# apple/ml-unigen

Measured on AMD Instinct MI355X. Metric: train-step samples/s (1.5B, 256^2 img), higher is better.
Workload: dtype bf16

## Files before the change

include/unigen_hip.h:

```cpp
#ifndef UNIGEN_HIP_H
#define UNIGEN_HIP_H

#include <stdint.h>
#include <hip/hip_runtime_api.h>

#ifdef __cplusplus
extern "C" {
#endif

#define UG_ABI_VERSION 7

const char* ug_last_error(void);
int ug_abi_version(void);

typedef struct ug_handle ug_handle;
int ug_create(ug_handle** out);
int ug_destroy(ug_handle* h);

#define UG_EPI_BF16 0
#define UG_EPI_F32 1
#define UG_EPI_RESID 2
int ug_gemm_bf16(const ug_handle* h, const void* A, int64_t lda, int a_kmajor, const void* B, int64_t ldb, int b_kmajor,
                 void* C, int64_t ldc, int64_t M, int64_t N, int64_t K, int epilogue, const void* bias,
                 const float* resid, int64_t ldr, int beta, const float* alpha_dev, int policy, hipStream_t stream);
#define UG_GEMM_NARROW_EPILOGUE 0x100
#define UG_GEMM_ONE_BARRIER 0x200
#define UG_GEMM_TWO_BARRIERS 0x400
#define UG_GEMM_POLICY_AUTO_BITS 0xff

int ug_cast_f32_bf16(const float* in, void* out, int64_t n, hipStream_t stream);

int ug_gemm_bf16_swiglu_bwd(const ug_handle* h, const void* dy, int64_t ld_dy, const void* w_down, int64_t ldw, const void* gu,
                            int64_t ld_gu, void* dgu, int64_t ld_dgu, int64_t M, int64_t I, int64_t K, hipStream_t stream);
int ug_gemm_set_fused_tile_height(int rows);
int ug_gemm_bf16_qkv_rope(const ug_handle* h, const void* x, int64_t ldx, const void* w, int64_t ldw, const void* bias, void* qkv,
                          int64_t ldq, int64_t M, int64_t N, int64_t K, const float* cos_tab, const float* sin_tab, int64_t L,
                          int64_t rope_cols, int head_dim, hipStream_t stream);
int ug_gemm_bf16_swiglu(const ug_handle* h, const void* x, int64_t ldx, const void* w_gate_up, int64_t ldw, void* gu,
                        int64_t ld_gu, void* act, int64_t ld_act, int64_t M, int64_t I, int64_t K, hipStream_t stream);

int ug_gemm_bf16_wgrad_group(int n, const void* const* dy, const int64_t* ld_dy, const void* const* x, const int64_t* ld_x,
                             float* const* dw, const int64_t* ld_dw, const int64_t* rows, const int64_t* cols,
                             const int* beta, const int64_t* K, hipStream_t stream);

int ug_rmsnorm_fwd(const float* x, const float* w, void* y, float* rstd, int64_t rows, int64_t cols,
                   float eps, int out_f32, hipStream_t stream);
int ug_rmsnorm_bwd(const void* dy, const float* x, const float* rstd, const float* w, float* dres,
                   float* dw, void* dres_bf16, int64_t rows, int64_t cols, hipStream_t stream);
int ug_rope(void* qkv, const float* cos_tab, const float* sin_tab, int64_t tokens, int64_t L, int64_t ldq,
            int nheads, int head_dim, int backward, hipStream_t stream);
int ug_swiglu_fwd(const void* gate_up, void* act, int64_t tokens, int64_t I, hipStream_t stream);
int ug_swiglu_bwd(const void* gate_up, const void* dact, void* dgate_up, int64_t tokens, int64_t I,
                  hipStream_t stream);
int ug_gelu(const void* x, const void* dy_or_null, void* out, int64_t n, hipStream_t stream);
int ug_embed_fwd(const int64_t* ids, const float* W, float* out, int64_t tokens, int64_t H, int64_t V,
                 int* err_flag, hipStream_t stream);
int ug_embed_bwd(const int64_t* ids, const float* dout, float* dW, int64_t tokens, int64_t H, int64_t V,
                 hipStream_t stream);
int ug_embed_bwd_sorted(const int64_t* ids_sorted, const int64_t* order, const float* rows, float* dW, int64_t n,
                        int64_t H, int64_t V, float scale, hipStream_t stream);
int ug_gather_rows_bf16(const void* in, int64_t ld_in, const int64_t* idx, void* out, int64_t ld_out,
                        int64_t n, int64_t C, int scatter, hipStream_t stream);
int ug_colsum_bf16(const void* in, int64_t ld, float* out, int64_t R, int64_t C, hipStream_t stream);

#define UG_MASK_F32 0
#define UG_MASK_BF16 1
#define UG_MASK_I64 2
// ... 215 lines not shown
```

ml-unigen_amd/csrc/gemm_bf16.hip:

```cpp
#include "common.h"
#include <type_traits>
#include <atomic>
#include "unigen_hip.h"
#include "vmem_asm.h"
#include "gemm_plan.h"

namespace {

using namespace ug_plan;
constexpr int TILE_BYTES = BM * BK * 2;
constexpr int GROUP_M = 8;
constexpr int P8_GROUP_M = 4;

typedef const __attribute__((address_space(1))) void* gptr_t;
typedef __attribute__((address_space(3))) void* lptr_t;
typedef __attribute__((ext_vector_type(4))) short s16x4_t;

__device__ __attribute__((aligned(16))) uint32_t g_zero_page[64];

struct GemmArgs {
  const bf16_t* A; const bf16_t* B; void* C;
  const bf16_t* bias;
  const float* resid;
  const float* alpha_dev;
  int M, N, K;
  int64_t lda, ldb, ldc, ldr;
  int beta;
  const bf16_t* sw_gu; int64_t ld_gu;
  const float* rope_cos; const float* rope_sin; int rope_L, rope_cols;
  int tiles_m, tiles_n;
  int full_tiles, tail_split;
  float* tail_ws;
  int tail_private;
  int one_barrier;
  int wide_epilogue;
  int swiglu_I;
  bf16_t* act; int64_t ld_act;
};
// ... 770 lines not shown
      if constexpr (decltype(steady)::value) {
        stage_in(t + 3);
        landed(2);
      } else {
        if (t + 3 < nk) stage_in(t + 3);
        landed(min(nk - 1, t + 3) - (t + 1));
      }
      asm volatile("s_waitcnt lgkmcnt(0)" ::: "memory");
      P_BARRIER();
      __builtin_amdgcn_s_setprio(1);
      UG_MFMA_BLOCK(FG)
      __builtin_amdgcn_s_setprio(0);
      P_BARRIER();
    };
    int t = 0;
    for (; t + 4 < nk; ++t) iteration(t, std::true_type{});
    for (; t < nk; ++t) iteration(t, std::false_type{});
    if (G0) P_BARRIER();
    if constexpr (EPI == EPI_SWIGLU_BWD)
      store_tile_swiglu_bwd<FG>(p, reinterpret_cast<f32x4_t (&)[FG][4]>(acc[0]), lds + wave * EP_STRIP, m0 + (G0 ? 0 : 16 * F0), n0 + wn * 64, lane);
    else if constexpr (EPI == EPI_SWIGLU)
      store_tile_swiglu_perm<FG>(p, reinterpret_cast<f32x4_t (&)[FG][4]>(acc[0]), lds + wave * EP_STRIP, m0 + (G0 ? 0 : 16 * F0), tn * 128 + wn * 32, lane);
    else if constexpr (EPI == EPI_ROPE)
      store_tile_lds<EPI, FG>(p, reinterpret_cast<f32x4_t (&)[FG][4]>(acc[0]), lds + wave * EP_STRIP, m0 + (G0 ? 0 : 16 * F0),
                              n0 + (wn >> 1) * 128 + (wn & 1) * 32, lane, (wn & 1) * 32, n0 < p.rope_cols);
    else
      store_tile_lds<EPI, FG>(p, reinterpret_cast<f32x4_t (&)[FG][4]>(acc[0]), lds + wave * EP_STRIP, m0 + (G0 ? 0 : 16 * F0), n0 + wn * 64, lane);
  };
  const bool more = REM != 0 && wave < REM;
  if (grp == 0) { if (more) run(std::true_type{}, std::integral_constant<int, LO + (REM ? 1 : 0)>{}); else run(std::true_type{}, std::integral_constant<int, LO>{}); }
  else { if (more) run(std::false_type{}, std::integral_constant<int, LO + (REM ? 1 : 0)>{}); else run(std::false_type{}, std::integral_constant<int, LO>{}); }
}


template <int EPI>
__global__ __launch_bounds__(256) void tail_finish_kernel(GemmArgs p, int ntail) {
  const int nwg = p.tiles_m * p.tiles_n;
  const int per_tile = PBM * PBN / 4;
  const int64_t total = (int64_t)ntail * per_tile;
  float alpha = 1.f;
  if constexpr (EPI == EPI_F32) { if (p.alpha_dev) alpha = *p.alpha_dev; }
  for (int64_t idx = blockIdx.x * (int64_t)blockDim.x + threadIdx.x; idx < total; idx += (int64_t)gridDim.x * blockDim.x) {
    const int tl = (int)(idx / per_tile), q = (int)(idx % per_tile);
    const int pid = xcd_remap(p.full_tiles + tl, nwg);
    const int per_group = P8_GROUP_M * p.tiles_n;
    const int gid = pid / per_group, first_m = gid * P8_GROUP_M;
    const int gsz = min(p.tiles_m - first_m, P8_GROUP_M);
    const int tm = first_m + (pid % per_group) % gsz;
    const int tn = (pid % per_group) / gsz;
    const int ml = q / (PBN / 4), nl = (q % (PBN / 4)) * 4;
    float4 v4;
    if (p.tail_private) {
      const int nk_all = (p.K + PBK - 1) / PBK, per_split = (nk_all + p.tail_split - 1) / p.tail_split;
      v4 = make_float4(0.f, 0.f, 0.f, 0.f);
      for (int sp = 0; sp < p.tail_split && sp * per_split < nk_all; ++sp) {
        const float4 t = *reinterpret_cast<const float4*>(p.tail_ws + ((int64_t)tl * p.tail_split + sp) * (PBM * PBN) + ml * PBN + nl);
        v4.x += t.x; v4.y += t.y; v4.z += t.z; v4.w += t.w;
      }
    } else {
      float4* src = reinterpret_cast<float4*>(p.tail_ws + (int64_t)tl * (PBM * PBN) + ml * PBN + nl);
      v4 = *src;
      *src = make_float4(0.f, 0.f, 0.f, 0.f);
    }
    const int m = tm * PBM + ml, n = tn * PBN + nl;
    if (m >= p.M || n >= p.N) continue;
    float v[4] = {v4.x, v4.y, v4.z, v4.w};
    for (int r = 0; r < 4 && n + r < p.N; ++r) {
      if constexpr (EPI == EPI_BF16) {
        float o = v[r];
        if (p.bias) o += bf2f(p.bias[n + r]);
        reinterpret_cast<bf16_t*>(p.C)[(int64_t)m * p.ldc + n + r] = f2bf(o);
      } else if constexpr (EPI == EPI_F32) {
        float* c = reinterpret_cast<float*>(p.C) + (int64_t)m * p.ldc + n + r;
        *c = (p.beta ? *c : 0.f) + v[r] * alpha;
      } else {
        reinterpret_cast<float*>(p.C)[(int64_t)m * p.ldc + n + r] = p.resid[(int64_t)m * p.ldr + n + r] + bf2f(f2bf(v[r]));
      }
    }
  }
}

static_assert(WS_PRIVATE_SLOTS == UG_HANDLE_WS_SLOTS && POLICY_NARROW_EPILOGUE == UG_GEMM_NARROW_EPILOGUE && POLICY_ONE_BARRIER == UG_GEMM_ONE_BARRIER &&
              POLICY_TWO_BARRIERS == UG_GEMM_TWO_BARRIERS && POLICY_AUTO_BITS == UG_GEMM_POLICY_AUTO_BITS, "gemm_plan.h restates these");

bool env_switch_on(const char* name) { const char* v = getenv(name); return !(v && atoi(v) == 0); }

template <int EPI, bool BKM, int H>
bool launch_p10_height(int height, dim3 grid, const GemmArgs& a, hipStream_t st) {
  if (height != H) return false;
  hipLaunchKernelGGL((gemm_kernel_p10<EPI, BKM, p10_f0(H), p10_f1(H)>), grid, dim3(512), 0, st, a);
  return true;
}
template <int EPI, bool BKM, int... H>
bool launch_p10(HeightList<H...>, int height, dim3 grid, const GemmArgs& a, hipStream_t st) {
  return (launch_p10_height<EPI, BKM, H>(height, grid, a, st) || ...);
}

template <int EPI, bool AK, bool BKM>
int run_plan(const GemmPlan& pl, GemmArgs a, hipStream_t st) {
  a.tiles_m = pl.tiles_m; a.tiles_n = pl.tiles_n;
  a.full_tiles = pl.full_tiles; a.tail_split = pl.tail_split; a.tail_private = pl.tail_private;
  if (!pl.uses_workspace) a.tail_ws = nullptr;
  const dim3 grid(pl.grid_x, pl.grid_y);
  if (pl.kind == KIND_P10) {
    if constexpr (!AK && EPI != EPI_F32) {
      if (launch_p10<EPI, BKM>(typename P10Heights<EPI>::type{}, pl.height, grid, a, st)) {
        UG_CHECK_LAUNCH("ug_gemm_bf16(p10)");
        return UG_OK;
      }
    }
    ug_set_error("ug_gemm_bf16: no %d-row tile kernel for this layout and epilogue", pl.height);
    return UG_ERR_ARG;
  }
  if (pl.kind == KIND_128) {
    if (pl.dbuf) hipLaunchKernelGGL((gemm_kernel<EPI, AK, BKM, true>), grid, dim3(256), 0, st, a);
    else hipLaunchKernelGGL((gemm_kernel<EPI, AK, BKM, false>), grid, dim3(256), 0, st, a);
    UG_CHECK_LAUNCH("ug_gemm_bf16");
    return UG_OK;
  }
  const bool sliced = pl.kind == KIND_256_SLICED;
  if (a.one_barrier) hipLaunchKernelGGL((gemm_kernel_p8<EPI, AK, BKM, true>), grid, dim3(512), 0, st, a);
  else hipLaunchKernelGGL((gemm_kernel_p8<EPI, AK, BKM>), grid, dim3(512), 0, st, a);
  UG_CHECK_LAUNCH(sliced ? "ug_gemm_bf16(p8 k-sliced)" : "ug_gemm_bf16(p8)");
  if (pl.finish_tiles) {
    hipLaunchKernelGGL((tail_finish_kernel<EPI>), dim3(pl.finish_tiles * 16), dim3(256), 0, st, a, pl.finish_tiles);
    UG_CHECK_LAUNCH(sliced ? "ug_gemm_bf16(partial sum)" : "ug_gemm_bf16(tail finish)");
  }
  return UG_OK;
}

std::atomic<int> g_fused_height{0};

template <int EPI, bool BKM>
int launch_fused(GemmArgs a, int64_t col_tiles, const char* who, hipStream_t st) {
  const int forced = g_fused_height.load();
  const int hb = plan_fused(EPI, a.M, col_tiles, forced);
  if (hb < 0) {
    ug_set_error("%s: tile height %d forced by ug_gemm_set_fused_tile_height is not instantiated for this epilogue", who, forced);
    return UG_ERR_ARG;
  }
  a.tiles_m = (a.M + hb - 1) / hb; a.tiles_n = (int)col_tiles;
  a.tail_split = 1; a.tail_private = 1; a.wide_epilogue = 1;
  launch_p10<EPI, BKM>(typename P10Heights<EPI>::type{}, hb, dim3(a.tiles_m * a.tiles_n), a, st);
  UG_CHECK_LAUNCH(who);
  return UG_OK;
}

}

extern "C" int ug_gemm_bf16(const ug_handle* h, const void* A, int64_t lda, int a_kmajor, const void* B, int64_t ldb, int b_kmajor,
                            void* C, int64_t ldc, int64_t M, int64_t N, int64_t K, int epilogue, const void* bias,
                            const float* resid, int64_t ldr, int beta, const float* alpha_dev, int policy, hipStream_t stream) {
  UG_REQUIRE(M > 0 && N > 0 && K > 0, "ug_gemm_bf16: empty problem M=%ld N=%ld K=%ld", (long)M, (long)N, (long)K);
  UG_REQUIRE(lda % 8 == 0 && ldb % 8 == 0, "ug_gemm_bf16: lda/ldb must be multiples of 8 elements (16-byte rows)");
  UG_REQUIRE(ug_aligned16(A) && ug_aligned16(B) && ug_aligned16(C), "ug_gemm_bf16: A/B/C must be 16-byte aligned");
  UG_REQUIRE(ldc % 4 == 0, "ug_gemm_bf16: ldc must be a multiple of 4 elements");
  UG_REQUIRE(M < (1 << 30) && N < (1 << 30) && K < (1 << 30), "ug_gemm_bf16: dims too large");
  UG_REQUIRE(a_kmajor || b_kmajor || K % 8 == 0,
             "ug_gemm_bf16: K=%ld must be a multiple of 8 when both operands are row-major", (long)K);
  UG_REQUIRE(a_kmajor || lda >= ((K + 7) & ~7LL), "ug_gemm_bf16: row-major A needs lda >= round_up(K,8)");
  UG_REQUIRE(b_kmajor || ldb >= ((K + 7) & ~7LL), "ug_gemm_bf16: row-major B needs ldb >= round_up(K,8)");
  UG_REQUIRE(!a_kmajor || lda >= M, "ug_gemm_bf16: k-major A needs lda >= M");
  UG_REQUIRE(!b_kmajor || ldb >= N, "ug_gemm_bf16: k-major B needs ldb >= N");
  if (epilogue == EPI_RESID) UG_REQUIRE(resid != nullptr && ldr % 4 == 0, "ug_gemm_bf16: EPI_RESID needs a 16B-aligned residual");
  const GemmPolicy pol = decode_policy(policy, a_kmajor != 0, b_kmajor != 0);
  GemmArgs a{};
  a.A = (const bf16_t*)A; a.B = (const bf16_t*)B; a.C = C;
  a.bias = (const bf16_t*)bias; a.resid = resid; a.alpha_dev = alpha_dev;
  a.M = (int)M; a.N = (int)N; a.K = (int)K;
  a.lda = lda; a.ldb = ldb; a.ldc = ldc; a.ldr = ldr; a.beta = beta;
  a.wide_epilogue = pol.wide_epilogue; a.one_barrier = pol.one_barrier;
  a.tail_ws = h ? h->tail_ws : nullptr;
  static const bool heights_on = env_switch_on("UNIGEN_GEMM_HEIGHTS");
  GemmProblem pr;
  pr.M = a.M; pr.N = a.N; pr.K = a.K; pr.epilogue = epilogue; pr.a_kmajor = a_kmajor != 0; pr.b_kmajor = b_kmajor != 0; pr.beta = beta;
  pr.ldc = ldc; pr.ldr = ldr; pr.bias_aligned8 = !bias || (reinterpret_cast<uintptr_t>(bias) & 7) == 0;
  pr.has_workspace = a.tail_ws != nullptr; pr.policy = pol.policy; pr.heights_on = heights_on;
  const GemmPlan pl = plan_gemm(pr);
  const int mode = (a_kmajor ? 2 : 0) | (b_kmajor ? 1 : 0);
  switch (mode * 4 + epilogue) {
    case 0 * 4 + EPI_BF16: return run_plan<EPI_BF16, false, false>(pl, a, stream);
    case 0 * 4 + EPI_F32: return run_plan<EPI_F32, false, false>(pl, a, stream);
    case 0 * 4 + EPI_RESID: return run_plan<EPI_RESID, false, false>(pl, a, stream);
    case 1 * 4 + EPI_BF16: return run_plan<EPI_BF16, false, true>(pl, a, stream);
    case 1 * 4 + EPI_F32: return run_plan<EPI_F32, false, true>(pl, a, stream);
    case 3 * 4 + EPI_F32: return run_plan<EPI_F32, true, true>(pl, a, stream);
    case 3 * 4 + EPI_BF16: return run_plan<EPI_BF16, true, true>(pl, a, stream);
    default:
      ug_set_error("ug_gemm_bf16: layout/epilogue combination (a_kmajor=%d b_kmajor=%d epilogue=%d) is not instantiated",
                   a_kmajor, b_kmajor, epilogue);
      return UG_ERR_ARG;
  }
}

extern "C" int ug_gemm_bf16_wgrad_group(int n, const void* const* dy, const int64_t* ld_dy, const void* const* x, const int64_t* ld_x,
                                        float* const* dw, const int64_t* ld_dw, const int64_t* rows, const int64_t* cols,
                                        const int* beta, const int64_t* K, hipStream_t stream) {
  UG_REQUIRE(n >= 1 && n <= GROUP_MAX && K, "ug_gemm_bf16_wgrad_group: 1..%d problems and their contraction lengths required", GROUP_MAX);
  GroupArgs g;
  g.n = n;
  int start = 0;
  for (int i = 0; i < n; ++i) {
    UG_REQUIRE(rows[i] > 0 && cols[i] > 0 && rows[i] < (1 << 30) && cols[i] < (1 << 30) && K[i] > 0 && K[i] < (1 << 30),
               "ug_gemm_bf16_wgrad_group: empty problem %d", i);
    UG_REQUIRE(ld_dy[i] % 8 == 0 && ld_x[i] % 8 == 0 && ld_dy[i] >= rows[i] && ld_x[i] >= cols[i] && ld_dw[i] % 4 == 0 && ld_dw[i] >= cols[i],
               "ug_gemm_bf16_wgrad_group: problem %d: token-major operands need leading dimensions that are multiples of 8 and cover "
               "their rows; ld_dw a multiple of 4", i);
    UG_REQUIRE(ug_aligned16(dy[i]) && ug_aligned16(x[i]) && ug_aligned16(dw[i]), "ug_gemm_bf16_wgrad_group: problem %d: 16-byte alignment", i);
    GroupProblem& pr = g.pr[i];
    pr.A = (const bf16_t*)dy[i]; pr.B = (const bf16_t*)x[i]; pr.C = dw[i];
    pr.lda = ld_dy[i]; pr.ldb = ld_x[i]; pr.ldc = ld_dw[i];
    pr.M = (int)rows[i]; pr.N = (int)cols[i]; pr.K = (int)K[i]; pr.beta = beta[i];
    pr.tiles_m = (pr.M + PBM - 1) / PBM; pr.tiles_n = (pr.N + PBN - 1) / PBN;
    pr.start = start;
    start += (pr.tiles_m * pr.tiles_n + 7) & ~7;
  }
  for (int i = n; i < GROUP_MAX; ++i) { g.pr[i] = g.pr[0]; g.pr[i].start = 1 << 30; }
  hipLaunchKernelGGL(gemm_kernel_p8_wgrad_group, dim3(start), dim3(512), 0, stream, g);
  UG_CHECK_LAUNCH("ug_gemm_bf16_wgrad_group");
  return UG_OK;
}

extern "C" int ug_gemm_set_fused_tile_height(int rows) {
  UG_REQUIRE(rows == 0 || (rows >= 128 && rows <= 320 && rows % 16 == 0), "ug_gemm_set_fused_tile_height: 0 (automatic) or 128 ... 320 in steps of 16 (%d)", rows);
  g_fused_height.store(rows);
  return UG_OK;
}

extern "C" int ug_swiglu_fwd(const void* gate_up, void* act, int64_t tokens, int64_t I, hipStream_t st);

extern "C" int ug_gemm_bf16_swiglu(const ug_handle* h, const void* x, int64_t ldx, const void* w_gate_up, int64_t ldw, void* gu,
                                   int64_t ld_gu, void* act, int64_t ld_act, int64_t M, int64_t I, int64_t K, hipStream_t stream) {
  UG_REQUIRE(M > 0 && I > 0 && K > 0 && K % 8 == 0 && I % 8 == 0, "ug_gemm_bf16_swiglu: bad problem M=%ld I=%ld K=%ld", (long)M, (long)I, (long)K);
  UG_REQUIRE(ldx % 8 == 0 && ldw % 8 == 0 && ld_gu % 8 == 0 && ld_act % 8 == 0 && ldx >= K && ldw >= K && ld_gu >= 2 * I && ld_act >= I,
             "ug_gemm_bf16_swiglu: row strides must be multiples of 8 elements and cover the rows");
  UG_REQUIRE(ug_aligned16(x) && ug_aligned16(w_gate_up) && ug_aligned16(gu) && ug_aligned16(act), "ug_gemm_bf16_swiglu: alignment");
  UG_REQUIRE(M < (1 << 30) && I < (1 << 29) && K < (1 << 30), "ug_gemm_bf16_swiglu: dims too large");
  const int64_t tiles = ((M + PBM - 1) / PBM) * (2 * I / PBN);
  if (I % 128 != 0 || tiles < 64 || K % PBK != 0 || 2 * I / PBN > (1 << 20)) {
    if (int rc = ug_gemm_bf16(h, x, ldx, 0, w_gate_up, ldw, 0, gu, ld_gu, M, 2 * I, K, EPI_BF16, nullptr, nullptr, 0, 0, nullptr, -1, stream))
      return rc;
    UG_REQUIRE(ld_gu == 2 * I && ld_act == I, "ug_gemm_bf16_swiglu: the two-launch form needs packed gu / act rows");
    return ug_swiglu_fwd(gu, act, M, I, stream);
  }
  GemmArgs a{};
  a.A = (const bf16_t*)x; a.B = (const bf16_t*)w_gate_up; a.C = gu;
  a.M = (int)M; a.N = (int)(2 * I); a.K = (int)K;
  a.lda = ldx; a.ldb = ldw; a.ldc = ld_gu;
  a.swiglu_I = (int)I; a.act = (bf16_t*)act; a.ld_act = ld_act;
  return launch_fused<EPI_SWIGLU, false>(a, 2 * I / PBN, "ug_gemm_bf16_swiglu", stream);
}

extern "C" int ug_rope(void* qkv, const float* cos_tab, const float* sin_tab, int64_t tokens, int64_t L, int64_t ldq,
                       int nheads, int head_dim, int backward, hipStream_t st);

extern "C" int ug_gemm_bf16_qkv_rope(const ug_handle* h, const void* x, int64_t ldx, const void* w, int64_t ldw, const void* bias, void* qkv,
                                     int64_t ldq, int64_t M, int64_t N, int64_t K, const float* cos_tab, const float* sin_tab, int64_t L,
                                     int64_t rope_cols, int head_dim, hipStream_t stream) {
  UG_REQUIRE(M > 0 && N > 0 && K > 0 && L > 0 && M % L == 0 && head_dim > 0 && rope_cols >= 0 && rope_cols <= N && rope_cols % head_dim == 0,
             "ug_gemm_bf16_qkv_rope: bad problem M=%ld N=%ld K=%ld L=%ld rope_cols=%ld head_dim=%d", (long)M, (long)N, (long)K, (long)L,
             (long)rope_cols, head_dim);
// ... 35 lines not shown
```

ml-unigen_amd/csrc/gemm_plan.h:

```cpp
#pragma once
#include <cstdint>

namespace ug_plan {

enum Epi { EPI_BF16 = 0, EPI_F32 = 1, EPI_RESID = 2, EPI_ROPE = 3, EPI_SWIGLU = 4, EPI_SWIGLU_BWD = 5 };

constexpr int BM = 128, BN = 128, BK = 64;
constexpr int PBM = 256, PBN = 256, PBK = 32;
constexpr int QBM = 320;
constexpr int WS_PRIVATE_SLOTS = 768;

constexpr int imin(int a, int b) { return a < b ? a : b; }
constexpr int imax(int a, int b) { return a > b ? a : b; }

constexpr int POLICY_NARROW_EPILOGUE = 0x100, POLICY_ONE_BARRIER = 0x200, POLICY_TWO_BARRIERS = 0x400, POLICY_AUTO_BITS = 0xff;

struct GemmPolicy {
  int policy;
  bool one_barrier;
  bool wide_epilogue;
};

inline GemmPolicy decode_policy(int policy, bool a_kmajor, bool b_kmajor) {
  GemmPolicy d;
  d.wide_epilogue = !(policy >= 0 && (policy & POLICY_NARROW_EPILOGUE));
  d.one_barrier = a_kmajor && b_kmajor;
  if (policy >= 0 && (policy & POLICY_ONE_BARRIER)) d.one_barrier = true;
  if (policy >= 0 && (policy & POLICY_TWO_BARRIERS)) d.one_barrier = false;
  if (policy >= 0) policy &= ~(POLICY_NARROW_EPILOGUE | POLICY_ONE_BARRIER | POLICY_TWO_BARRIERS);
  if (policy == POLICY_AUTO_BITS) policy = -1;
  d.policy = policy;
  return d;
}

constexpr int p10_f0(int h) { return (h / 16 + 1) / 2; }
constexpr int p10_f1(int h) { return (h / 16) / 2; }

template <int... H>
struct HeightList {
  static constexpr int count = sizeof...(H);
  static constexpr int values[sizeof...(H)] = {H...};
};
template <int EPI> struct P10Heights { using type = HeightList<128, 144, 160, 176, 192, 208, 224, 240, 256, 272, 288, 304, 320>; };
template <> struct P10Heights<EPI_ROPE> { using type = HeightList<128, 160, 192, 208, 224, 256, 288, 320>; };
template <> struct P10Heights<EPI_SWIGLU> { using type = HeightList<128, 160, 192, 208, 224, 256, 288, 320>; };
template <> struct P10Heights<EPI_SWIGLU_BWD> { using type = HeightList<128, 160, 192, 208, 224, 256, 272, 288, 320>; };

struct GemmProblem {
  int M, N, K;
  int epilogue;
  bool a_kmajor, b_kmajor;
  int beta;
  int64_t ldc, ldr;
  bool bias_aligned8;
  bool has_workspace;
  int policy;
  bool heights_on;
};

enum GemmKind { KIND_128 = 0, KIND_256 = 1, KIND_256_SLICED = 2, KIND_P10 = 3 };

struct GemmPlan {
// ... 140 lines not shown
```

ml-unigen_amd/unigen_hip/lib.py:

```python
import ctypes
import os
import subprocess

_HERE = os.path.dirname(os.path.abspath(__file__))
CSRC_DIR = os.path.normpath(os.path.join(_HERE, "..", "csrc"))
LIB_PATH = os.environ.get("UNIGEN_HIP_LIB") or os.path.join(CSRC_DIR, "libunigen_hip.so")

ABI_VERSION = 7
P = ctypes.c_void_p
I64 = ctypes.c_int64
I32 = ctypes.c_int
F32 = ctypes.c_float

SIGNATURES = {
    "ug_abi_version": [],
    "ug_create": [P],
    "ug_destroy": [P],
    "ug_gemm_bf16": [P, P, I64, I32, P, I64, I32, P, I64, I64, I64, I64, I32, P, P, I64, I32, P, I32, P],
    "ug_gemm_bf16_qkv_rope": [P, P, I64, P, I64, P, P, I64, I64, I64, I64, P, P, I64, I64, I32, P],
    "ug_gemm_bf16_swiglu_bwd": [P, P, I64, P, I64, P, I64, P, I64, I64, I64, I64, P],
    "ug_gemm_bf16_swiglu": [P, P, I64, P, I64, P, I64, P, I64, I64, I64, I64, P],
    "ug_cast_f32_bf16": [P, P, I64, P],
    "ug_rmsnorm_fwd": [P, P, P, P, I64, I64, F32, I32, P],
    "ug_rmsnorm_bwd": [P, P, P, P, P, P, P, I64, I64, P],
    "ug_rope": [P, P, P, I64, I64, I64, I32, I32, I32, P],
    "ug_swiglu_fwd": [P, P, I64, I64, P],
    "ug_swiglu_bwd": [P, P, P, I64, I64, P],
    "ug_gelu": [P, P, P, I64, P],
    "ug_embed_fwd": [P, P, P, I64, I64, I64, P, P],
    "ug_embed_bwd": [P, P, P, I64, I64, I64, P],
    "ug_embed_bwd_sorted": [P, P, P, P, I64, I64, I64, F32, P],
    "ug_gather_rows_bf16": [P, I64, P, P, I64, I64, I64, I32, P],
    "ug_colsum_bf16": [P, I64, P, I64, I64, P],
    "ug_attn_mask_compress": [P, I32, I64, I64, P, P, I64, I64, P, P],
    "ug_attn_mask_causal": [P, P, P, I64, I64, P],
    "ug_attn_fwd": [P, P, P, I64, P, I64, P, P, P, I64, I64, I64, I32, I32, I32, F32, P],
    "ug_attn_bwd": [P, P, P, I64, P, P, I64, P, P, P, P, P, I64, P, P, I64, I64, I64, I32, I32, I32, F32, P, P, P, P, P],
    "ug_kv_store": [P, I64, I64, I64, P, P, I64, I64, I32, I32, I64, P, I32, P],
    "ug_rope_at": [P, P, P, I64, I64, I32, I32, P, I64, P],
    "ug_attn_decode": [P, I64, P, P, P, P, I64, I64, I32, I32, I32, I64, P, F32, P],
    "ug_gemv_bf16": [P, I64, I64, P, I64, P, I64, I64, I64, I64, P],
    "ug_decode_gemv": [P, I64, I64, P, I64, P, I64, I64, I64, P, I64, P, I64, P, P],
    "ug_decode_gemv_resid_norm": [P, P, I64, P, P, P, I64, P, I64, P, I64, I64, I64, P, I64, P, I64, P, P],
    "ug_decode_gemv_swiglu": [P, I64, P, F32, I64, I64, P, I64, P, I64, I64, I64, P, I64, P, I64, P, P],
    "ug_gemm_set_fused_tile_height": [I32],
    "ug_attn_decode_fused": [P, I64, P, F32, I64, P, P, P, P, P, P, P, P, I64, I64, I32, I32, I32, I64, I64, F32, P],
    "ug_decode_finish_resid_norm": [P, I64, P, P, P, I64, I64, F32, P, P, P],
    "ug_decode_sw_supported": [I64, I64, I64, I32],
    "ug_decode_sw_kblock": [P, I64, I64, P, I64, P, I64, I64, I64, P, I64, P, I64, P, P],
    "ug_decode_sw_resid": [P, I64, I64, P, I64, I64, I64, P, P],
    "ug_decode_sw_gate_up": [P, P, I64, P, P, F32, I64, I64, P, I64, I64, P, I64, P],
    "ug_decode_sw_head": [P, P, I64, P, P, F32, I64, I64, P, I64, I64, P, I64, P, P, P],
    "ug_t2i_assemble": [P, P, P, I64, P, I64, P, P, I64, I64, I64, I64, I64, I64, I64, P, P, P, P],
    "ug_attn_mask_from_ids": [P, I64, I64, I64, I64, I64, I32, P, P, P, P, P],
    "ug_maskgit_train_mask": [P, P, P, I64, I64, I64, I64, P, P, P],
    "ug_ar_sample": [P, I64, I64, I64, F32, F32, I32, P, P, I64, I64, P, I64, I64, I64, P, P, P, P],
    "ug_ar_sample_filtered": [P, I64, I64, I64, F32, F32, I32, P, P, I64, I64, P, I64, I64, I64, P, P, P, I64, F32, F32, P, P],
    "ug_text_pick": [P, I64, I64, I64, I32, P, I64, I64, P, I64, I64, I64, P, I64, P, P, P, P, P],
    "ug_text_sample_workspace_ints": [I64],
    "ug_text_sample": [P, I64, I64, I64, I32, F32, I64, F32, P, P, P, P, I64, I64, P, I64, I64, I64, P, I64, P, P, P, P, P],
    "ug_ar_sample_logp": [P, I64, I64, I64, F32, F32, I32, P, P, I64, I64, P, I64, I64, I64, P, P, P, P, P],
    "ug_ar_sample_filtered_logp": [P, I64, I64, I64, F32, F32, I32, P, P, I64, I64, P, I64, I64, I64, P, P, P, I64, F32, F32, P, P, P],
    "ug_text_pick_logp": [P, I64, I64, I64, I32, P, I64, I64, P, I64, I64, I64, P, I64, P, P, P, P, P, P],
    "ug_text_sample_logp": [P, I64, I64, I64, I32, F32, I64, F32, P, P, P, P, I64, I64, P, I64, I64, I64, P, I64, P, P, P, P, P, P],
    "ug_text_seen_mark": [P, I64, P, I64, I64, I64, P, I64, P],
    "ug_text_penalize": [P, I64, I64, I64, F32, P, I64, P, P],
    "ug_maskgit_step": [P, I64, I64, I64, I64, I32, F32, P, P, P, I64, I64, I64, F32, P, P, P, P, P, P],
    "ug_skinny_finish": [P, P, P, P, I64, I64, I32, P],
    "ug_gemv_bf16_ord": [P, I64, I64, P, I64, P, I64, I64, I64, I64, P],
    "ug_skinny_finish_ord": [P, I64, I64, P, P, P, P, I64, I64, P],
    "ug_decode_gemv_resid_norm_ord": [P, P, I64, I64, P, P, P, I64, P, I64, P, I64, I64, I64, P],
    "ug_attn_decode_fused_ord": [P, I64, I64, P, F32, I64, P, P, P, P, P, P, P, P, I64, I64, I32, I32, I32, I64, I64, F32, P],
    "ug_decode_sw_kblock_ord": [P, I64, I64, P, I64, P, I64, I64, I64, P],
    "ug_decode_finish_resid_norm_ord": [P, I64, I64, P, P, P, I64, I64, F32, P, P, P],
    "ug_ce_fwd": [P, I64, I64, I64, P, I64, P, P, P, P, P],
    "ug_ce_bwd": [P, I64, I64, I64, P, I64, P, P, P, P, P],
    "ug_adamw_flat": [P, P, P, P, P, I64, F32, F32, F32, F32, F32, I64, F32, I32, P],
    "ug_gemm_bf16_wgrad_group": [I32, P, P, P, P, P, P, P, P, P, P, P],
# ... 130 lines not shown
```

ml-unigen_amd/unigen_hip/ops.py:

```python
import contextlib
import ctypes
import math
import torch

from . import lib as _l

UG_EPI_BF16, UG_EPI_F32, UG_EPI_RESID = 0, 1, 2
_MASK_DTYPES = {torch.float32: 0, torch.bfloat16: 1, torch.int64: 2, torch.bool: 3}


GEMM_PROFILE = None
GEMM_PROFILE_FUSED = None


class _GemmTimed:

    def __init__(self, prof, flops, fused):
        self.prof, self.flops, self.fused = prof, flops, fused

    def __enter__(self):
        self.e0, self.e1 = torch.cuda.Event(enable_timing=True), torch.cuda.Event(enable_timing=True)
        self.e0.record()

    def __exit__(self, exc_type, exc, tb):
        if exc_type is None:
            self.e1.record()
            self.prof.append((self.e0, self.e1, self.flops))
            if self.fused and GEMM_PROFILE_FUSED is not None:
                GEMM_PROFILE_FUSED.append(len(self.prof) - 1)
        return False


_UNTIMED = contextlib.nullcontext()


def _gemm_timed(flops, fused=False):
    prof = GEMM_PROFILE
    return _UNTIMED if prof is None else _GemmTimed(prof, flops, fused)


def _stream():
    return torch.cuda.current_stream().cuda_stream


def _p(t):
    return 0 if t is None else t.data_ptr()


_HANDLES = {}
GEMM_POLICY = -1
UG_GEMM_NARROW_EPILOGUE, UG_GEMM_POLICY_AUTO_BITS = 0x100, 0xff


def _handle():
    s = torch.cuda.current_stream()
    key = (s.device_index, s.cuda_stream)
    h = _HANDLES.get(key)
    if h is None:
        if torch.cuda.is_current_stream_capturing():
            return 0
        out = ctypes.c_void_p()
        _l.check(_l.load().ug_create(ctypes.byref(out)), "ug_create")
        h = _HANDLES[key] = out.value
    return h


def release_handles():
    lib = _l.load()
    for h in _HANDLES.values():
        lib.ug_destroy(h)
    _HANDLES.clear()


def _need_cuda(*ts):
    for t in ts:
        if t is not None and not t.is_cuda:
            raise _l.UniGenHipError("unigen_hip ops need tensors in GPU memory (no CPU fallback exists)")


def round_up(x, m):
    return (x + m - 1) // m * m


def gemm(a, b, out=None, *, M=None, N=None, K=None, a_kmajor=False, b_kmajor=False, epilogue=UG_EPI_BF16,
# ... 46 lines not shown
        return
    n = len(problems)
    PA, LA, IA = ctypes.c_void_p * n, ctypes.c_int64 * n, ctypes.c_int * n
    for dy, x, dw, _ in problems:
        _need_cuda(dy, x, dw)
        assert dy.shape[0] == x.shape[0] and dw.shape == (dy.shape[1], x.shape[1])
    with _gemm_timed(sum(2.0 * dy.shape[1] * x.shape[1] * dy.shape[0] for dy, x, _, _ in problems)):
        rc = _l.load().ug_gemm_bf16_wgrad_group(
            n, PA(*[_p(dy) for dy, _, _, _ in problems]), LA(*[dy.stride(0) for dy, _, _, _ in problems]),
            PA(*[_p(x) for _, x, _, _ in problems]), LA(*[x.stride(0) for _, x, _, _ in problems]),
            PA(*[_p(dw) for _, _, dw, _ in problems]), LA(*[dw.stride(0) for _, _, dw, _ in problems]),
            LA(*[dy.shape[1] for dy, _, _, _ in problems]), LA(*[x.shape[1] for _, x, _, _ in problems]),
            IA(*[int(b) for _, _, _, b in problems]), LA(*[dy.shape[0] for dy, _, _, _ in problems]), _stream())
        _l.check(rc, "ug_gemm_bf16_wgrad_group")


def set_gemm_tile_policy(policy):
    global GEMM_POLICY
    policy = int(policy)
    if policy == 100:
        GEMM_POLICY = UG_GEMM_POLICY_AUTO_BITS | UG_GEMM_NARROW_EPILOGUE
    elif policy == 101:
        GEMM_POLICY = -1
    elif policy in (102, 104):
        GEMM_POLICY = UG_GEMM_POLICY_AUTO_BITS | (0x200 if policy == 102 else 0x400)
    elif policy in (103, 105):
        GEMM_POLICY = 3 | (0x200 if policy == 103 else 0x400)
    else:
        GEMM_POLICY = policy


def set_fused_tile_height(rows):
    _l.check(_l.load().ug_gemm_set_fused_tile_height(int(rows)), "ug_gemm_set_fused_tile_height")


def gemm_nt(a, b, out=None, **kw):
    return gemm(a, b, out, **kw)


def cast_bf16(x, out=None):
    _need_cuda(x)
    if out is None:
        out = torch.empty(x.shape, dtype=torch.bfloat16, device=x.device)
    _l.check(_l.load().ug_cast_f32_bf16(_p(x), _p(out), x.numel(), _stream()), "ug_cast_f32_bf16")
    return out


def zero_ranges_(buf, ranges, max_len):
    _l.check(_l.load().ug_zero_ranges_f32(_p(buf), _p(ranges), ranges.shape[0], int(max_len), _stream()), "ug_zero_ranges_f32")
    return buf


def grad_pack_bf16(g, out, scale):
    _need_cuda(g, out)
    _l.check(_l.load().ug_grad_pack_bf16(_p(g), _p(out), g.numel(), float(scale), _stream()), "ug_grad_pack_bf16")


def grad_unpack_bf16(src, g):
    _need_cuda(src, g)
    _l.check(_l.load().ug_grad_unpack_bf16(_p(src), _p(g), g.numel(), _stream()), "ug_grad_unpack_bf16")


def grad_sum_shards_bf16(shards, world, stride, out, scale):
    _need_cuda(shards, out)
    _l.check(_l.load().ug_grad_sum_shards_bf16(_p(shards), int(world), int(stride), _p(out), out.numel(), float(scale), _stream()),
             "ug_grad_sum_shards_bf16")
# ... 901 lines not shown
```

Before: 131.0.

## Stage GEMM operands as full 128-byte lines across K-tile pairs

Adds a p10 GEMM kernel variant that loads A and (for non-k-major B) B in 128-byte row lines covering two 32-wide K tiles at once. The data goes into a swizzled, double-buffered LDS pair layout, so each global load is a full cache line instead of a 64-byte half. This variant becomes the default for eligible aligned shapes. A policy bit and a setter keep the old 64-byte staging reachable. The cost is a new pipeline schedule with different waitcnt accounting, a tail path for odd K-tile counts, and more LDS for the A region.

```diff
diff --git a/include/unigen_hip.h b/include/unigen_hip.h
--- a/include/unigen_hip.h
+++ b/include/unigen_hip.h
@@ -26,6 +26,7 @@
 #define UG_GEMM_NARROW_EPILOGUE 0x100
 #define UG_GEMM_ONE_BARRIER 0x200
 #define UG_GEMM_TWO_BARRIERS 0x400
+#define UG_GEMM_STAGE_64B 0x800
 #define UG_GEMM_POLICY_AUTO_BITS 0xff
 
 int ug_cast_f32_bf16(const float* in, void* out, int64_t n, hipStream_t stream);
@@ -33,6 +34,7 @@
 int ug_gemm_bf16_swiglu_bwd(const ug_handle* h, const void* dy, int64_t ld_dy, const void* w_down, int64_t ldw, const void* gu,
                             int64_t ld_gu, void* dgu, int64_t ld_dgu, int64_t M, int64_t I, int64_t K, hipStream_t stream);
 int ug_gemm_set_fused_tile_height(int rows);
+int ug_gemm_set_fused_staging(int line_bytes);
 int ug_gemm_bf16_qkv_rope(const ug_handle* h, const void* x, int64_t ldx, const void* w, int64_t ldw, const void* bias, void* qkv,
                           int64_t ldq, int64_t M, int64_t N, int64_t K, const float* cos_tab, const float* sin_tab, int64_t L,
                           int64_t rope_cols, int head_dim, hipStream_t stream);
diff --git a/ml-unigen_amd/csrc/gemm_bf16.hip b/ml-unigen_amd/csrc/gemm_bf16.hip
--- a/ml-unigen_amd/csrc/gemm_bf16.hip
+++ b/ml-unigen_amd/csrc/gemm_bf16.hip
@@ -4,6 +4,7 @@
 #include "unigen_hip.h"
 #include "vmem_asm.h"
 #include "gemm_plan.h"
+#include "gemm_stage64.h"
 
 namespace {
 
@@ -840,6 +841,174 @@
   else { if (more) run(std::false_type{}, std::integral_constant<int, LO + (REM ? 1 : 0)>{}); else run(std::false_type{}, std::integral_constant<int, LO>{}); }
 }
 
+template <int EPI, bool BKM, int F0, int F1>
+__global__ __launch_bounds__(512, 2) void gemm_kernel_p10s(GemmArgs p) {
+  namespace s64 = ug_stage64;
+  constexpr int BMV = 16 * (F0 + F1), NP = BMV / 8, LO = NP / 8, REM = NP % 8;
+  constexpr int PAIR_A = BMV * s64::PITCH, B_REGION = 2 * PAIR_A, PAIR_B = PBN * s64::PITCH;
+  static_assert(F0 >= F1 && F0 <= 10 && F1 >= 1 && LO >= 2 && LO + (REM ? 1 : 0) <= 5, "gemm_kernel_p10s: unsupported tile height");
+  static_assert(2 * PAIR_B == P_NST * P_TILE, "both B layouts fill the same region");
+  __shared__ __attribute__((aligned(16))) char lds[B_REGION + P_NST * P_TILE];
+  const int tid = threadIdx.x, lane = tid & 63;
+  const int wave = __builtin_amdgcn_readfirstlane(tid >> 6);
+  const int grp = wave >> 2, wn = wave & 3;
+  const int nwg = p.tiles_m * p.tiles_n;
+  const int pid = xcd_remap((int)blockIdx.x, nwg);
+  const int per_group = P10_GROUP_M * p.tiles_n;
+  const int gid = pid / per_group, first_m = gid * P10_GROUP_M;
+  const int gsz = min(p.tiles_m - first_m, P10_GROUP_M);
+  const int tm = first_m + (pid % per_group) % gsz;
+  const int tn = (pid % per_group) / gsz;
+  const int m0 = tm * BMV, n0 = tn * PBN;
+
+  const int chunk = s64::src_chunk(wave, lane, false);
+  const uint32_t tailsub = (uint32_t)(chunk - s64::src_chunk(wave, lane, true)) * 16;
+  uint32_t aoff[5];
+#pragma unroll
+  for (int i = 0; i < 5; ++i) {
+    const int piece = min(i * 8 + wave, NP - 1);
+    aoff[i] = s64::lane_offset(min(m0 + s64::piece_row(piece, lane), p.M - 1) - m0, p.lda, chunk);
+  }
+  const uint64_t abase = reinterpret_cast<uint64_t>(p.A + (int64_t)m0 * p.lda);
+  uint32_t boff[4] = {0u, 0u, 0u, 0u};
+  uint64_t bbase = 0;
+  if constexpr (BKM) {
+#pragma unroll
+    for (int i = 0; i < 2; ++i) {
+      const int k = (i * 8 + wave) * 2 + (lane >> 5);
+      boff[i] = (uint32_t)(((int64_t)k * p.ldb + swz_krow(k, lane & 31) * 8) * 2);
+    }
+    bbase = reinterpret_cast<uint64_t>(p.B + n0);
+  } else {
+    const int brow0 = EPI == EPI_SWIGLU ? tn * 128 : n0;
+#pragma unroll
+    for (int i = 0; i < 4; ++i) {
+      const int row = s64::piece_row(i * 8 + wave, lane);
+      const int grow = (EPI == EPI_SWIGLU && row >= 128) ? p.swiglu_I + brow0 + row - 128 : brow0 + row;
+      boff[i] = s64::lane_offset(min(grow, p.N - 1) - brow0, p.ldb, chunk);
+    }
+    bbase = reinterpret_cast<uint64_t>(p.B + (int64_t)brow0 * p.ldb);
+  }
+  const int foff0 = s64::frag_offset(0, 0, lane);
+
+  f32x4_t acc[F0][4];
+#pragma unroll
+  for (int i = 0; i < F0; ++i)
+#pragma unroll
+    for (int j = 0; j < 4; ++j) acc[i][j] = f32x4_t{0.f, 0.f, 0.f, 0.f};
+  const int nk = p.K / PBK;
+  const int npairs = s64::num_pairs(nk);
+
+  auto run = [&](auto group0, auto nap_tag) {
+    constexpr bool G0 = decltype(group0)::value;
+    constexpr int NAP = decltype(nap_tag)::value;
+    constexpr int FG = G0 ? F0 : F1;
+    auto issue_pair = [&](int D, uint32_t sub) {
+      const uint64_t ab = abase + s64::pair_offset(D);
+      char* sa = lds + (D & 1) * PAIR_A;
+#pragma unroll
+      for (int i = 0; i < NAP; ++i)
+        dma16(ab, aoff[i] - sub, __builtin_amdgcn_readfirstlane(lds_addr_of(sa + (i * 8 + wave) * s64::PIECE_BYTES)));
+      if constexpr (!BKM) {
+        const uint64_t bb = bbase + s64::pair_offset(D);
+        char* sbp = lds + B_REGION + (D & 1) * PAIR_B;
+#pragma unroll
+        for (int i = 0; i < 4; ++i)
+          dma16(bb, boff[i] - sub, __builtin_amdgcn_readfirstlane(lds_addr_of(sbp + (i * 8 + wave) * s64::PIECE_BYTES)));
+      }
+    };
+    auto issue_b = [&](int lt) {
+      if constexpr (BKM) {
+        const uint64_t bb = bbase + (int64_t)lt * PBK * p.ldb * 2;
+        char* st = lds + B_REGION + (lt & (P_NST - 1)) * P_TILE;
+#pragma unroll
+        for (int i = 0; i < 2; ++i) dma16(bb, boff[i], __builtin_amdgcn_readfirstlane(lds_addr_of(st + (i * 8 + wave) * 1024)));
+      }
+    };
+    auto wait_allow = [&](int n) {
+#define UG_W(v) case v: asm volatile("s_waitcnt vmcnt(" #v ")" ::: "memory"); break;
+      switch (n) {
+        UG_W(1) UG_W(2) UG_W(3) UG_W(4) UG_W(5) UG_W(6) UG_W(7) UG_W(8) UG_W(9)
+        default: asm volatile("s_waitcnt vmcnt(0)" ::: "memory"); break;
+      }
+#undef UG_W
+    };
+    issue_pair(0, s64::pair_is_tail(0, nk) ? tailsub : 0u);
+    if constexpr (BKM) {
+      issue_b(0);
+      if (nk > 1) issue_b(1);
+      if (nk > 2) issue_b(2);
+      wait_allow(2 * (min(nk, 3) - 1));
+    } else {
+      wait_allow(0);
+    }
+    P_BARRIER();
+    if (!G0) P_BARRIER();
+    auto iteration = [&](int t, auto mode) {
+      constexpr int MODE = decltype(mode)::value;
+      const int slot = (t >> 1) & 1;
+      const int foff = foff0 ^ ((t & 1) << 6);
+      const char* tA = lds + slot * PAIR_A + (G0 ? 0 : 16 * F0) * s64::PITCH + foff;
+      bf16x8_t fa[FG], fb[4];
+#pragma unroll
+      for (int i = 0; i < FG; ++i) fa[i] = *reinterpret_cast<const bf16x8_t*>(tA + i * 16 * s64::PITCH);
+#pragma unroll
+      for (int j = 0; j < 4; ++j) {
+        const int rb = EPI == EPI_ROPE ? (wn >> 1) * 128 + (wn & 1) * 32 + (j & 1) * 16 + (j >> 1) * 64
+                       : EPI == EPI_SWIGLU ? (j >> 1) * 128 + wn * 32 + (j & 1) * 16 : wn * 64 + j * 16;
+        if constexpr (BKM) fb[j] = load_frag32<true>(lds + B_REGION + (t & (P_NST - 1)) * P_TILE, rb, lane);
+        else fb[j] = *reinterpret_cast<const bf16x8_t*>(lds + B_REGION + slot * PAIR_B + rb * s64::PITCH + foff);
+      }
+      if constexpr (MODE == 0) {
+        issue_pair((t >> 1) + 1, 0u);
+        issue_b(t + 3);
+        if constexpr (BKM) asm volatile("s_waitcnt vmcnt(%0)" ::"n"(NAP + 4) : "memory");
+      } else if constexpr (MODE == 1) {
+        issue_b(t + 3);
+        if constexpr (BKM) asm volatile("s_waitcnt vmcnt(4)" ::: "memory");
+        else asm volatile("s_waitcnt vmcnt(0)" ::: "memory");
+      } else {
+        const int b2 = (BKM && t + 2 < nk) ? 2 : 0, b3 = (BKM && t + 3 < nk) ? 2 : 0;
+        if (!(t & 1)) {
+          const int D = (t >> 1) + 1;
+          const int a = D < npairs ? NAP + (BKM ? 0 : 4) : 0;
+          if (a) issue_pair(D, s64::pair_is_tail(D, nk) ? tailsub : 0u);
+          if (b3) issue_b(t + 3);
+          if (BKM || t + 1 >= nk) wait_allow(t + 1 < nk ? b2 + a + b3 : 0);
+        } else {
+          if (b3) issue_b(t + 3);
+          wait_allow(t + 1 < nk ? b2 + b3 : 0);
+        }
+      }
+      asm volatile("s_waitcnt lgkmcnt(0)" ::: "memory");
+      P_BARRIER();
+      __builtin_amdgcn_s_setprio(1);
+      UG_MFMA_BLOCK(FG)
+      __builtin_amdgcn_s_setprio(0);
+      P_BARRIER();
+    };
+    int t = 0;
+    for (; t + 4 < nk; t += 2) {
+      iteration(t, std::integral_constant<int, 0>{});
+      iteration(t + 1, std::integral_constant<int, 1>{});
+    }
+    for (; t < nk; ++t) iteration(t, std::integral_constant<int, 2>{});
+    if (G0) P_BARRIER();
+    if constexpr (EPI == EPI_SWIGLU_BWD)
+      store_tile_swiglu_bwd<FG>(p, reinterpret_cast<f32x4_t (&)[FG][4]>(acc[0]), lds + wave * EP_STRIP, m0 + (G0 ? 0 : 16 * F0), n0 + wn * 64, lane);
+    else if constexpr (EPI == EPI_SWIGLU)
+      store_tile_swiglu_perm<FG>(p, reinterpret_cast<f32x4_t (&)[FG][4]>(acc[0]), lds + wave * EP_STRIP, m0 + (G0 ? 0 : 16 * F0), tn * 128 + wn * 32, lane);
+    else if constexpr (EPI == EPI_ROPE)
+      store_tile_lds<EPI, FG>(p, reinterpret_cast<f32x4_t (&)[FG][4]>(acc[0]), lds + wave * EP_STRIP, m0 + (G0 ? 0 : 16 * F0),
+                              n0 + (wn >> 1) * 128 + (wn & 1) * 32, lane, (wn & 1) * 32, n0 < p.rope_cols);
+    else
+      store_tile_lds<EPI, FG>(p, reinterpret_cast<f32x4_t (&)[FG][4]>(acc[0]), lds + wave * EP_STRIP, m0 + (G0 ? 0 : 16 * F0), n0 + wn * 64, lane);
+  };
+  const bool more = REM != 0 && wave < REM;
+  if (grp == 0) { if (more) run(std::true_type{}, std::integral_constant<int, LO + (REM ? 1 : 0)>{}); else run(std::true_type{}, std::integral_constant<int, LO>{}); }
+  else { if (more) run(std::false_type{}, std::integral_constant<int, LO + (REM ? 1 : 0)>{}); else run(std::false_type{}, std::integral_constant<int, LO>{}); }
+}
+
 
 template <int EPI>
 __global__ __launch_bounds__(256) void tail_finish_kernel(GemmArgs p, int ntail) {
@@ -889,30 +1058,47 @@
 }
 
 static_assert(WS_PRIVATE_SLOTS == UG_HANDLE_WS_SLOTS && POLICY_NARROW_EPILOGUE == UG_GEMM_NARROW_EPILOGUE && POLICY_ONE_BARRIER == UG_GEMM_ONE_BARRIER &&
-              POLICY_TWO_BARRIERS == UG_GEMM_TWO_BARRIERS && POLICY_AUTO_BITS == UG_GEMM_POLICY_AUTO_BITS, "gemm_plan.h restates these");
+              POLICY_TWO_BARRIERS == UG_GEMM_TWO_BARRIERS && POLICY_STAGE_64B == UG_GEMM_STAGE_64B && POLICY_AUTO_BITS == UG_GEMM_POLICY_AUTO_BITS, "gemm_plan.h restates these");
 
 bool env_switch_on(const char* name) { const char* v = getenv(name); return !(v && atoi(v) == 0); }
 
+constexpr bool line_staging_default(int epi, bool bkm) { (void)epi; return !bkm; }
+
+template <int EPI, bool BKM>
+bool use_line_staging(const GemmArgs& a, int height, bool wanted) {
+  namespace s64 = ug_stage64;
+  return wanted && line_staging_default(EPI, BKM) && s64::eligible(reinterpret_cast<uintptr_t>(a.A), a.lda, height) &&
+         (BKM ? a.ldb * (2 * PBK * 2) < ((int64_t)1 << 32)
+              : s64::eligible(reinterpret_cast<uintptr_t>(a.B), a.ldb, a.N));
+}
+
 template <int EPI, bool BKM, int H>
-bool launch_p10_height(int height, dim3 grid, const GemmArgs& a, hipStream_t st) {
+bool launch_p10_height(int height, dim3 grid, const GemmArgs& a, bool lines, hipStream_t st) {
   if (height != H) return false;
+  if constexpr (line_staging_default(EPI, BKM)) {
+    if (lines) {
+      hipLaunchKernelGGL((gemm_kernel_p10s<EPI, BKM, p10_f0(H), p10_f1(H)>), grid, dim3(512), 0, st, a);
+      return true;
+    }
+  }
   hipLaunchKernelGGL((gemm_kernel_p10<EPI, BKM, p10_f0(H), p10_f1(H)>), grid, dim3(512), 0, st, a);
   return true;
 }
 template <int EPI, bool BKM, int... H>
-bool launch_p10(HeightList<H...>, int height, dim3 grid, const GemmArgs& a, hipStream_t st) {
-  return (launch_p10_height<EPI, BKM, H>(height, grid, a, st) || ...);
+bool launch_p10(HeightList<H...>, int height, dim3 grid, const GemmArgs& a, bool lines_wanted, hipStream_t st) {
+  const bool lines = use_line_staging<EPI, BKM>(a, height, lines_wanted);
+  return (launch_p10_height<EPI, BKM, H>(height, grid, a, lines, st) || ...);
 }
 
 template <int EPI, bool AK, bool BKM>
-int run_plan(const GemmPlan& pl, GemmArgs a, hipStream_t st) {
+int run_plan(const GemmPlan& pl, GemmArgs a, bool line_staging, hipStream_t st) {
   a.tiles_m = pl.tiles_m; a.tiles_n = pl.tiles_n;
   a.full_tiles = pl.full_tiles; a.tail_split = pl.tail_split; a.tail_private = pl.tail_private;
   if (!pl.uses_workspace) a.tail_ws = nullptr;
   const dim3 grid(pl.grid_x, pl.grid_y);
   if (pl.kind == KIND_P10) {
     if constexpr (!AK && EPI != EPI_F32) {
-      if (launch_p10<EPI, BKM>(typename P10Heights<EPI>::type{}, pl.height, grid, a, st)) {
+      if (launch_p10<EPI, BKM>(typename P10Heights<EPI>::type{}, pl.height, grid, a, line_staging, st)) {
         UG_CHECK_LAUNCH("ug_gemm_bf16(p10)");
         return UG_OK;
       }
@@ -938,6 +1124,7 @@
 }
 
 std::atomic<int> g_fused_height{0};
+std::atomic<int> g_fused_line_bytes{128};
 
 template <int EPI, bool BKM>
 int launch_fused(GemmArgs a, int64_t col_tiles, const char* who, hipStream_t st) {
@@ -949,7 +1136,7 @@
   }
   a.tiles_m = (a.M + hb - 1) / hb; a.tiles_n = (int)col_tiles;
   a.tail_split = 1; a.tail_private = 1; a.wide_epilogue = 1;
-  launch_p10<EPI, BKM>(typename P10Heights<EPI>::type{}, hb, dim3(a.tiles_m * a.tiles_n), a, st);
+  launch_p10<EPI, BKM>(typename P10Heights<EPI>::type{}, hb, dim3(a.tiles_m * a.tiles_n), a, g_fused_line_bytes.load() == 128, st);
   UG_CHECK_LAUNCH(who);
   return UG_OK;
 }
@@ -987,13 +1174,13 @@
   const GemmPlan pl = plan_gemm(pr);
   const int mode = (a_kmajor ? 2 : 0) | (b_kmajor ? 1 : 0);
   switch (mode * 4 + epilogue) {
-    case 0 * 4 + EPI_BF16: return run_plan<EPI_BF16, false, false>(pl, a, stream);
-    case 0 * 4 + EPI_F32: return run_plan<EPI_F32, false, false>(pl, a, stream);
-    case 0 * 4 + EPI_RESID: return run_plan<EPI_RESID, false, false>(pl, a, stream);
-    case 1 * 4 + EPI_BF16: return run_plan<EPI_BF16, false, true>(pl, a, stream);
-    case 1 * 4 + EPI_F32: return run_plan<EPI_F32, false, true>(pl, a, stream);
-    case 3 * 4 + EPI_F32: return run_plan<EPI_F32, true, true>(pl, a, stream);
-    case 3 * 4 + EPI_BF16: return run_plan<EPI_BF16, true, true>(pl, a, stream);
+    case 0 * 4 + EPI_BF16: return run_plan<EPI_BF16, false, false>(pl, a, pol.line_staging, stream);
+    case 0 * 4 + EPI_F32: return run_plan<EPI_F32, false, false>(pl, a, pol.line_staging, stream);
+    case 0 * 4 + EPI_RESID: return run_plan<EPI_RESID, false, false>(pl, a, pol.line_staging, stream);
+    case 1 * 4 + EPI_BF16: return run_plan<EPI_BF16, false, true>(pl, a, pol.line_staging, stream);
+    case 1 * 4 + EPI_F32: return run_plan<EPI_F32, false, true>(pl, a, pol.line_staging, stream);
+    case 3 * 4 + EPI_F32: return run_plan<EPI_F32, true, true>(pl, a, pol.line_staging, stream);
+    case 3 * 4 + EPI_BF16: return run_plan<EPI_BF16, true, true>(pl, a, pol.line_staging, stream);
     default:
       ug_set_error("ug_gemm_bf16: layout/epilogue combination (a_kmajor=%d b_kmajor=%d epilogue=%d) is not instantiated",
                    a_kmajor, b_kmajor, epilogue);
@@ -1035,6 +1222,12 @@
   return UG_OK;
 }
 
+extern "C" int ug_gemm_set_fused_staging(int line_bytes) {
+  UG_REQUIRE(line_bytes == 64 || line_bytes == 128, "ug_gemm_set_fused_staging: 128 (whole lines, the default) or 64 (%d)", line_bytes);
+  g_fused_line_bytes.store(line_bytes);
+  return UG_OK;
+}
+
 extern "C" int ug_swiglu_fwd(const void* gate_up, void* act, int64_t tokens, int64_t I, hipStream_t st);
 
 extern "C" int ug_gemm_bf16_swiglu(const ug_handle* h, const void* x, int64_t ldx, const void* w_gate_up, int64_t ldw, void* gu,
diff --git a/ml-unigen_amd/csrc/gemm_plan.h b/ml-unigen_amd/csrc/gemm_plan.h
--- a/ml-unigen_amd/csrc/gemm_plan.h
+++ b/ml-unigen_amd/csrc/gemm_plan.h
@@ -13,12 +13,13 @@
 constexpr int imin(int a, int b) { return a < b ? a : b; }
 constexpr int imax(int a, int b) { return a > b ? a : b; }
 
-constexpr int POLICY_NARROW_EPILOGUE = 0x100, POLICY_ONE_BARRIER = 0x200, POLICY_TWO_BARRIERS = 0x400, POLICY_AUTO_BITS = 0xff;
+constexpr int POLICY_NARROW_EPILOGUE = 0x100, POLICY_ONE_BARRIER = 0x200, POLICY_TWO_BARRIERS = 0x400, POLICY_STAGE_64B = 0x800, POLICY_AUTO_BITS = 0xff;
 
 struct GemmPolicy {
   int policy;
   bool one_barrier;
   bool wide_epilogue;
+  bool line_staging;
 };
 
 inline GemmPolicy decode_policy(int policy, bool a_kmajor, bool b_kmajor) {
@@ -27,7 +28,8 @@
   d.one_barrier = a_kmajor && b_kmajor;
   if (policy >= 0 && (policy & POLICY_ONE_BARRIER)) d.one_barrier = true;
   if (policy >= 0 && (policy & POLICY_TWO_BARRIERS)) d.one_barrier = false;
-  if (policy >= 0) policy &= ~(POLICY_NARROW_EPILOGUE | POLICY_ONE_BARRIER | POLICY_TWO_BARRIERS);
+  d.line_staging = !(policy >= 0 && (policy & POLICY_STAGE_64B));
+  if (policy >= 0) policy &= ~(POLICY_NARROW_EPILOGUE | POLICY_ONE_BARRIER | POLICY_TWO_BARRIERS | POLICY_STAGE_64B);
   if (policy == POLICY_AUTO_BITS) policy = -1;
   d.policy = policy;
   return d;
diff --git a/ml-unigen_amd/csrc/gemm_stage64.h b/ml-unigen_amd/csrc/gemm_stage64.h
--- /dev/null
+++ b/ml-unigen_amd/csrc/gemm_stage64.h
@@ -0,0 +1,41 @@
+#pragma once
+#include <cstdint>
+
+#if defined(__HIPCC__)
+#define UG_S64_FN __host__ __device__ inline
+#else
+#define UG_S64_FN inline
+#endif
+
+namespace ug_stage64 {
+
+constexpr int PAIR_K = 64;
+constexpr int PITCH = 128;
+constexpr int PIECE_ROWS = 8;
+constexpr int PIECE_BYTES = 1024;
+
+UG_S64_FN int swz(int row, int chunk) { return chunk ^ ((row >> 1) & 7); }
+
+UG_S64_FN int piece_row(int piece, int lane) { return piece * PIECE_ROWS + (lane >> 3); }
+UG_S64_FN int piece_pos(int lane) { return lane & 7; }
+UG_S64_FN int lds_offset(int piece, int lane) { return piece * PIECE_BYTES + lane * 16; }
+UG_S64_FN int src_chunk(int piece, int lane, bool tail) {
+  const int c = swz(piece_row(piece, lane), piece_pos(lane));
+  return tail ? (c & 3) : c;
+}
+UG_S64_FN uint32_t lane_offset(int rel_row, int64_t ld, int chunk) { return (uint32_t)((int64_t)rel_row * ld * 2 + chunk * 16); }
+UG_S64_FN int64_t pair_offset(int pair) { return (int64_t)pair * (PAIR_K * 2); }
+
+UG_S64_FN int frag_offset(int row0, int half, int lane) {
+  const int row = row0 + (lane & 15);
+  return row * PITCH + swz(row, 4 * half + (lane >> 4)) * 16;
+}
+
+UG_S64_FN bool eligible(uint64_t base_addr, int64_t ld, int64_t span_rows) {
+  return ld > 0 && ld % 64 == 0 && base_addr % 128 == 0 && span_rows * ld * 2 + PITCH < ((int64_t)1 << 32);
+}
+
+UG_S64_FN int num_pairs(int nk_tiles) { return (nk_tiles + 1) / 2; }
+UG_S64_FN bool pair_is_tail(int pair, int nk_tiles) { return (nk_tiles & 1) && pair == nk_tiles / 2; }
+
+}
diff --git a/ml-unigen_amd/unigen_hip/lib.py b/ml-unigen_amd/unigen_hip/lib.py
--- a/ml-unigen_amd/unigen_hip/lib.py
+++ b/ml-unigen_amd/unigen_hip/lib.py
@@ -44,6 +44,7 @@
     "ug_decode_gemv_resid_norm": [P, P, I64, P, P, P, I64, P, I64, P, I64, I64, I64, P, I64, P, I64, P, P],
     "ug_decode_gemv_swiglu": [P, I64, P, F32, I64, I64, P, I64, P, I64, I64, I64, P, I64, P, I64, P, P],
     "ug_gemm_set_fused_tile_height": [I32],
+    "ug_gemm_set_fused_staging": [I32],
     "ug_attn_decode_fused": [P, I64, P, F32, I64, P, P, P, P, P, P, P, P, I64, I64, I32, I32, I32, I64, I64, F32, P],
     "ug_decode_finish_resid_norm": [P, I64, P, P, P, I64, I64, F32, P, P, P],
     "ug_decode_sw_supported": [I64, I64, I64, I32],
diff --git a/ml-unigen_amd/unigen_hip/ops.py b/ml-unigen_amd/unigen_hip/ops.py
--- a/ml-unigen_amd/unigen_hip/ops.py
+++ b/ml-unigen_amd/unigen_hip/ops.py
@@ -50,6 +50,7 @@
 _HANDLES = {}
 GEMM_POLICY = -1
 UG_GEMM_NARROW_EPILOGUE, UG_GEMM_POLICY_AUTO_BITS = 0x100, 0xff
+UG_GEMM_STAGE_64B = 0x800
 
 
 def _handle():
@@ -162,6 +163,10 @@
 
 def set_fused_tile_height(rows):
     _l.check(_l.load().ug_gemm_set_fused_tile_height(int(rows)), "ug_gemm_set_fused_tile_height")
+
+
+def set_fused_staging(line_bytes):
+    _l.check(_l.load().ug_gemm_set_fused_staging(int(line_bytes)), "ug_gemm_set_fused_staging")
 
 
 def gemm_nt(a, b, out=None, **kw):
```

Measured after the change: 132.0 (median of 6 runs). No clear change (+0.8%).
